# kakaobrain/hqtransformer

Hardware: AMD Instinct MI355X
Metric: images/sec (256x256 class-cond sampling) (higher is better)
Workload: dtype bf16

## Files before the change

hqtransformer_amd/_lib.py:

```python
from __future__ import annotations

import ctypes as C
import os
import subprocess
from typing import List, Optional

HERE = os.path.dirname(os.path.abspath(__file__))
LIB_PATH = os.path.join(HERE, 'libhqt.so')
CSRC = os.path.join(HERE, 'csrc')
SOURCES = ['engine.hip', 'kernels.hip', 'attention.hip', 'fast_kernels.hip', 'persist.hip', 'tile_gemm.hip', 'exact_gemm.hip', 'mfma_gemm.hip', 'split_conv.hip', 'split_stream_conv.hip']
ABI_VERSION = 9

PRECISION_EXACT, PRECISION_FAST, PRECISION_SPLIT = 0, 1, 2
PRECISIONS = {'exact': PRECISION_EXACT, 'fast': PRECISION_FAST, 'split': PRECISION_SPLIT}
POLICY_LATENCY, POLICY_THROUGHPUT = 0, 1
SWITCH_PERSIST, SWITCH_SINGLE_KEY, SWITCH_PERSIST_FAULT, SWITCH_SPLIT_KSLICES = 0, 1, 2, 3
LAYOUT_FAST, LAYOUT_EXACT, LAYOUT_SPLIT, LAYOUT_ALL = 1, 2, 4, 7
RESAMPLE_PIXELSHUFFLE, RESAMPLE_NEAREST, RESAMPLE_CONV2 = 0, 1, 2


class HqtLibraryError(RuntimeError):
    pass


class HqtError(RuntimeError):
    def __init__(self, code: int, msg: str):
        super().__init__(f'libhqt error {code}: {msg}')
        self.code = code


class hqt_config(C.Structure):
# ... 78 lines not shown
    'hqt_decode_seq': (C.c_int, [_VP, C.c_int, _I64P, _I64P, _F32P, C.c_int, C.c_int, _VP]),
    'hqt_sample_l3': (C.c_int, [_VP, C.c_int, _I64P, C.POINTER(hqt_sample_opts_l3), _F32P, _I64P, _I64P, _I64P, _F32P, _I64P, _I64P, _I64P, _VP]),
    'hqt_sample_prefix_l3': (C.c_int, [_VP, C.c_int, _I64P, C.POINTER(hqt_sample_opts_l3), _F32P, C.c_int, _I64P, _I64P, _I64P, _I64P, _I64P, _I64P, _F32P, _I64P, _I64P, _I64P, _VP]),
    'hqt_decode_l3': (C.c_int, [_VP, C.c_int, _I64P, _I64P, _I64P, _F32P, C.c_int, C.c_int, _VP]),
    'hqt_decode_seq_l3': (C.c_int, [_VP, C.c_int, _I64P, _I64P, _I64P, _F32P, C.c_int, C.c_int, _VP]),
    'hqt_encode': (C.c_int, [_VP, C.c_int, _F32P, C.c_int, C.POINTER(hqt_encode_out), _VP]),
    'hqt_has_encoder': (C.c_int, [_VP]),
    'hqt_range_check': (C.c_int, [_VP, _VP]),
    'hqt_param_count': (C.c_int64, [_VP, C.c_int]),
    'hqt_workspace_bytes': (C.c_int64, [_VP]),
    'hqt_timing_enable': (C.c_int, [_VP, C.c_int]),
    'hqt_timing_reset': (C.c_int, [_VP]),
    'hqt_timing_get': (C.c_int, [_VP, C.c_int, C.c_char_p, C.c_int, C.POINTER(C.c_int64), C.POINTER(C.c_double)]),
    'hqt_timing_slots': (C.c_int, [_VP]),
    'hqt_destroy': (C.c_int, [_VP]),
}

_lib: Optional[C.CDLL] = None


def build(force: bool = False, verbose: bool = False) -> str:
    import hashlib
    from concurrent.futures import ThreadPoolExecutor
    hdrs = sorted([os.path.join(CSRC, f) for f in os.listdir(CSRC) if f.endswith('.h')] + [os.path.join(os.path.dirname(HERE), 'include', 'hqt.h')])
    hipcc = os.environ.get('HIPCC', '/opt/rocm/bin/hipcc')
    flags = ['-O3', '--offload-arch=gfx950', '-std=c++17', '-fPIC', '-Wno-unused-value', '-Wno-unused-result']
    objdir = os.path.join(CSRC, 'build')
    os.makedirs(objdir, exist_ok=True)
    ver = subprocess.run([hipcc, '--version'], stdout=subprocess.PIPE, stderr=subprocess.STDOUT, text=True).stdout
    common = hashlib.sha256()
# ... 134 lines not shown
```

hqtransformer_amd/csrc/common.h:

```cpp
#pragma once
#include <hip/hip_runtime.h>
#include <stdint.h>
#include <string>

typedef uint16_t bf16_t;

__device__ __host__ inline float bf16_to_f32(bf16_t v) {
    union { uint32_t u; float f; } c;
    c.u = ((uint32_t)v) << 16;
    return c.f;
}
__device__ __forceinline__ void bf16x8_to_f32(const uint4& raw, float (&f)[8]) {
    const unsigned w[4] = {raw.x, raw.y, raw.z, raw.w};
#pragma unroll
    for (int i = 0; i < 4; ++i) { f[2 * i] = bf16_to_f32((bf16_t)(w[i] & 0xffffu)); f[2 * i + 1] = bf16_to_f32((bf16_t)(w[i] >> 16)); }
}
__device__ __host__ inline bf16_t f32_to_bf16(float f) {
#if defined(__HIP_DEVICE_COMPILE__)
    return __builtin_bit_cast(bf16_t, (__bf16)f);
#endif
    union { uint32_t u; float f; } c;
    c.f = f;
    if ((c.u & 0x7fffffffu) > 0x7f800000u) return (bf16_t)((c.u >> 16) | 0x40);
    return (bf16_t)((c.u + 0x7fffu + ((c.u >> 16) & 1u)) >> 16);
// ... 104 lines not shown
    const float* ln_colsum;
    float ln_eps;
    bf16_t* resid_pk;
    float* resid_parts;
    unsigned* tile_ctr;
    const float* am_rownorm;
    const float* am_colnorm;
    unsigned long long* am_best;
    ChainSync chain;
    float* gn_part_out;
    int gn_out_groups;
    int tune;
    const void* Bw_lo;
    const void* Bw_frag16;
    const void* Bw_up16;
    double* gn_part_out_d;
    int a_f32;
    int b_f32;
    int* range_flag;
    int out_split;
    int k_quarters;
    int b_tile16;
    int k_slices;
    float* k_slabs;
    int tile_panel;
};

struct StepState {
    int step;
    int t_base;
// ... 19 lines not shown
```

hqtransformer_amd/csrc/engine.hip:

```cpp
#include "../../include/hqt.h"
#include "kernels.h"
#include "fast_kernels.h"
#include "split_kernels.h"
#include "persist.h"

#include <algorithm>
#include <cmath>
#include <cstdarg>
#include <cstdio>
#include <cstring>
#include <map>
#include <memory>
#include <mutex>
#include <string>
#include <vector>

static thread_local std::string g_err;
static int fail(int code, const char* fmt, ...) {
    char buf[1024];
    va_list ap;
    va_start(ap, fmt);
    vsnprintf(buf, sizeof(buf), fmt, ap);
    va_end(ap);
    g_err = buf;
// ... 28 lines not shown
struct Tensor {
    float* d = nullptr;
    std::vector<int64_t> shape;
    size_t n = 0;
};

struct Lin {
    const float* w32 = nullptr;
    const float* b32 = nullptr;
    bf16_t* w16 = nullptr;
    half_t* w16h = nullptr;
    half_t* w16l = nullptr;
    float* w32t = nullptr;
    half_t* wfrag16 = nullptr;
    half_t* wup16 = nullptr;
    bf16_t* wpk = nullptr;
    bf16_t* wpk_ln = nullptr;
    float* colsum = nullptr;
    float* bias_ln = nullptr;
    int N = 0, K = 0;
};

struct BlockW {
    bool body = false;
    const float *ln1_g, *ln1_b, *ln2_g, *ln2_b;
    Lin qkv, proj, fc1, fc2;
};

struct DecLayer {
    int kind;
// ... 88 lines not shown
    hipGraphExec_t graph_exec = nullptr;
    std::vector<uint64_t> graph_key;
    hqt_handle* parent = nullptr;
    int n_clones = 0;
    int policy = 0;
    PersistProg pbody, pfull;
    float* lnf_shift = nullptr;
    int ncu = 0;
    unsigned* persist_counters = nullptr;
    unsigned* persist_err = nullptr;
    float* persist_slabs = nullptr;
    bool persist_used = false;
    bool persist_enabled = true;
    bool persist_tripped = false;
    bool single_key = true;
    bool split_kslices = true;
    bool capture_persist = false;
    bool graph_has_persist = false;
    int layouts = 0;
    bool timing = false;
    std::vector<TimingSlot> slots;
    hipEvent_t chain_ev = nullptr;
    bool chain_valid = false;
    std::vector<hipEvent_t> all_events;
};

static int dev_alloc(hqt_handle* h, void** p, size_t bytes, bool workspace) {
    HIPCHK(hipMalloc(p, bytes ? bytes : 16));
    const bool poison = getenv("HQT_POISON_WORKSPACE") != nullptr;
    if (poison && workspace && bytes) HIPCHK(hipMemset(*p, 0xFF, bytes));
// ... 141 lines not shown
extern "C" const char* hqt_last_error(void) { return g_err.c_str(); }

static int alloc_workspace(hqt_handle* hp);

extern "C" int hqt_create(const hqt_config* cfg, int device, hqt_handle** out) {
    if (!cfg || !out) return fail(HQT_ERR_INVALID, "null argument");
    if (cfg->abi_version != HQT_ABI_VERSION) return fail(HQT_ERR_INVALID, "abi_version %d != %d", cfg->abi_version, HQT_ABI_VERSION);
    if (cfg->max_batch < 1) return fail(HQT_ERR_INVALID, "max_batch must be >= 1");
    DeviceGuard dg(device);
    if (!dg.ok) return fail(HQT_ERR_HIP, "hipSetDevice(%d) failed", device);
    std::unique_ptr<hqt_handle> h(new hqt_handle());
    h->tile_gemm = getenv("HQT_NO_TILE_GEMM") == nullptr;
    { const char* e = getenv("HQT_PERSIST"); h->persist_enabled = !(e && atoi(e) == 0); }
    h->single_key = getenv("HQT_NO_SINGLE_KEY") == nullptr;
    h->split_kslices = getenv("HQT_SPLIT_KSLICES_OFF") == nullptr;
    h->cfg = *cfg;
    h->layouts = (cfg->ar_layouts & HQT_LAYOUT_ALL) ? (cfg->ar_layouts & HQT_LAYOUT_ALL) : HQT_LAYOUT_ALL;
    h->device = device;
    const hqt_config& c = h->cfg;
    if (c.has_stage2) {
        if (c.embed_dim % c.n_heads || c.embed_dim % 16) return fail(HQT_ERR_INVALID, "embed_dim must be a multiple of n_heads and 16");
        const int hs = c.embed_dim / c.n_heads;
        if (hs % 8 || hs > 256 || (hs & (hs - 1))) return fail(HQT_ERR_INVALID, "head_dim %d unsupported (power of two in [8, 256])", hs);
        if (c.vocab_top != c.vocab_bot) return fail(HQT_ERR_INVALID, "vocab_top != vocab_bot");
        const bool bidir = c.depth_decoding == HQT_DEPTH_BIDIRECTIONAL;
        if (c.depth_decoding < 0 || c.depth_decoding > HQT_DEPTH_BIDIRECTIONAL || (c.depth_decoding && !bidir && c.code_levels != 3) || (bidir && c.code_levels == 3))
            return fail(HQT_ERR_INVALID, "depth_decoding %d: 0 'parallel-add', 1 'parallel', 2 'parallel-reduce', 3 'top2mid2bot' (three code levels only), "
                        "4 'bidirectional' (two code levels only)", c.depth_decoding);
        if (bidir && c.cond_type == HQT_COND_TEXT)
            return fail(HQT_ERR_INVALID, "depth_decoding 4 'bidirectional' with text conditioning is not built");
// ... 278 lines not shown
    *out = it->second.d;
    return HQT_OK;
}

static int make_lin(hqt_handle* h, Lin& l, const float* w32, const float* b32, int N, int K, bool stream_pack, bool split_planes = false) {
    l.w32 = w32; l.b32 = b32; l.N = N; l.K = K;
    if (!stream_pack || (h->layouts & HQT_LAYOUT_FAST)) {
        CHK(dev_alloc(h, (void**)&l.w16, (size_t)N * K * 2, false));
        HIPCHK(launch_f32_to_bf16(w32, l.w16, (size_t)N * K, 0));
    }
    const bool ar = stream_pack;
    if (split_planes && (!ar || (h->layouts & HQT_LAYOUT_SPLIT))) {
        CHK(dev_alloc(h, (void**)&l.w16h, (size_t)N * K * 2, false));
        CHK(dev_alloc(h, (void**)&l.w16l, (size_t)N * K * 2, false));
        HIPCHK(launch_split_f32(w32, l.w16h, l.w16l, (size_t)N * K, 0));
    }
    if (stream_pack && (h->layouts & HQT_LAYOUT_EXACT) && N % 16 == 0 && K % 32 == 0) {
        CHK(dev_alloc(h, (void**)&l.w32t, (size_t)N * K * 4, false));
        HIPCHK(launch_pack_exact_tiles(w32, l.w32t, N, K, 0));
    }
    if (stream_pack && (h->layouts & HQT_LAYOUT_FAST) && stream_gemm_supported(N, K)) {
        CHK(dev_alloc(h, (void**)&l.wpk, (size_t)N * K * 2, false));
        HIPCHK(launch_pack_stream_weights(w32, l.wpk, N, K, 0));
    }
    return HQT_OK;
}

static int fold_ln(hqt_handle* h, Lin& l, const float* gamma, const float* beta) {
    if (!l.wpk) return HQT_OK;
    CHK(dev_alloc(h, (void**)&l.wpk_ln, (size_t)l.N * l.K * 2, false));
// ... 241 lines not shown
            else if (l.kind == 1) {
                CHK(get_w(h, "stage1." + l.name + ".norm1.weight", {l.cin}, &l.n1_g));
                CHK(get_w(h, "stage1." + l.name + ".norm1.bias", {l.cin}, &l.n1_b));
                CHK(get_w(h, "stage1." + l.name + ".norm2.weight", {l.cout}, &l.n2_g));
                CHK(get_w(h, "stage1." + l.name + ".norm2.bias", {l.cout}, &l.n2_b));
                CHK(load_conv(h, l.name + ".conv1", l.cout, l.cin, 3, l.conv1));
                CHK(load_conv(h, l.name + ".conv2", l.cout, l.cout, 3, l.conv2));
                if (l.cin != l.cout) CHK(load_conv(h, l.name + ".nin_shortcut", l.cout, l.cin, 1, l.nin));
            } else if (l.kind == 2) {
                CHK(get_w(h, "stage1." + l.name + ".norm.weight", {l.cin}, &l.n1_g));
                CHK(get_w(h, "stage1." + l.name + ".norm.bias", {l.cin}, &l.n1_b));
                CHK(load_conv(h, l.name + ".q", l.cin, l.cin, 1, l.q));
                CHK(load_conv(h, l.name + ".k", l.cin, l.cin, 1, l.k));
                CHK(load_conv(h, l.name + ".v", l.cin, l.cin, 1, l.v));
                CHK(load_conv(h, l.name + ".proj_out", l.cin, l.cin, 1, l.proj));
            } else {
                CHK(get_w(h, "stage1.decoder.norm_out.weight", {l.cin}, &l.n1_g));
                CHK(get_w(h, "stage1.decoder.norm_out.bias", {l.cin}, &l.n1_b));
                CHK(load_conv(h, "decoder.conv_out", l.cout, l.cin, 3, l.conv1));
            }
        }
    }
    if (c.has_stage1 && h->w.count("stage1.encoder.conv_in.weight") && (c.s1_resample != HQT_RESAMPLE_CONV2 || h->w.count("stage1.down_t.weight")))
        CHK(load_encoder(h));
    HIPCHK(stream_gemm_configure());
    HIPCHK(tile_gemm_configure());
    HIPCHK(mfma_gemm_configure());
    HIPCHK(split_kernels_configure());
    HIPCHK(hipDeviceSynchronize());
    h->finalized = true;
    return HQT_OK;
// ... 9 lines not shown
static int mode_of(int precision, bool stage1, Mode* md) {
    if (precision == HQT_PRECISION_FAST) md->fast = true;
    else if (precision == HQT_PRECISION_SPLIT && stage1) md->split = true;
    else if (precision == HQT_PRECISION_SPLIT) md->split_ar = true;
    else if (precision != HQT_PRECISION_EXACT) return fail(HQT_ERR_INVALID, "unknown precision %d", precision);
    return HQT_OK;
}

static void lin_args(const hqt_handle* h, GemmArgs& g, const Lin& l, bool split_planes) {
    g.N = l.N; g.K = l.K; g.ldb = l.K;
    g.bias = l.b32;
    g.zero_page = h->zero_page;
    g.tune = h->policy;
    if (g.alpha == 0.0f) g.alpha = 1.0f;
    if (g.lda == 0) g.lda = l.K;
    if (split_planes) { g.Bw = l.w16h; g.Bw_lo = l.w16l; g.Bw_frag16 = l.wfrag16; g.Bw_up16 = l.wup16; }
}

struct SlotName {
    char s[64];
    SlotName(const char* tag, int rows) {
        static const bool by_rows = getenv("HQT_TIMING_BY_ROWS") != nullptr;
        snprintf(s, sizeof s, by_rows ? "%s@%d" : "%s", tag, rows);
    }
};

static int ar_linear(hqt_handle* h, const Mode& md, GemmArgs g, const Lin& l, int a_dt, int c_dt, hipStream_t st,
                     const char* tag, bool defer_residual = false, int* resid_nparts = nullptr) {
    lin_args(h, g, l, false);
    g.k_quarters = 1;
    const SlotName slot(tag, g.M);
// ... 28 lines not shown
            count_variant(h, "variant:stream_gemm:%s", tag);
            if (S > 1) h->pend = {h->splitk, S, 32 * g.a_packed_mb, l.b32};
            return HQT_OK;
        }
        g.Bw = l.w16;
        if (mfma_gemm_ok(g, a_dt, DT_BF16, c_dt)) HIPCHK(launch_mfma_gemm(g, a_dt, DT_BF16, c_dt, st));
        else HIPCHK(launch_gemm_generic(g, a_dt, DT_BF16, c_dt, st));
        return HQT_OK;
    }
    if (md.split_ar && l.w16h && l.w16l && !g.a_packed_mb && g.M > 256) {
        GemmArgs sg = g;
        lin_args(h, sg, l, true);
        sg.a_f32 = 1; sg.range_flag = h->range_flag;
        if (split_gemm_ok(sg)) {
            const int S = h->split_kslices ? split_gemm_slices(sg) : 1;
            if (S > 1 && (size_t)S * sg.M * sg.N <= h->splitk_elems) { sg.k_slices = S; sg.k_slabs = h->splitk; }
            HIPCHK(launch_split_gemm(sg, st));
            if (sg.k_slices > 1) count_variant(h, "variant:split_gemm_kslices%d:%s", sg.k_slices, tag);
            else count_variant(h, "variant:split_gemm:%s", tag);
            return HQT_OK;
        }
    }
    g.Bw = l.w32;
    if (exact_mfma_ok(g)) {
        if (l.w32t && g.N % 16 == 0) { g.Bw = l.w32t; g.b_tile16 = 1; }
        HIPCHK(launch_exact_mfma_gemm(g, st));
        count_variant(h, "variant:exact_mfma:%s", tag);
        return HQT_OK;
    }
    HIPCHK(launch_gemm_generic(g, DT_F32, DT_F32, DT_F32, st));
// ... 853 lines not shown
            Timed t(h, "embed_prefix", c.st);
            HIPCHK(launch_embed_prefix(embed_args(h, c, own), P + 1, P + 1, 0, 0, c.st));
        }
        CHK(run_position(h, c, P + 1, 0, false));
        HIPCHK(launch_advance_step(h->state, P + 1, c.st));
        first = P + 1;
    }
    const int remaining = c.n_steps - first;
    if (remaining <= 0) return HQT_OK;
    if (c.use_graph && !h->timing) {
        static const int gmax = getenv("HQT_GRAPH_POSITIONS") ? std::max(1, atoi(getenv("HQT_GRAPH_POSITIONS"))) : 16;
        int G = 1;
        for (int d = std::min(gmax, remaining); d >= 1; --d) if (remaining % d == 0) { G = d; break; }
        std::vector<uint64_t> key = {(uint64_t)G, (uint64_t)B, (uint64_t)(c.cond != nullptr), (uint64_t)c.noise, (uint64_t)c.logits_out, (uint64_t)c.logprob_out,
                                     (uint64_t)c.precision, (uint64_t)c.n_steps, (uint64_t)c.levels, (uint64_t)h->policy,
                                     (uint64_t)((h->persist_enabled && !h->persist_tripped ? 1 : 0) + (h->single_key ? 0 : 4) + (h->split_kslices ? 0 : 8))};
        for (const int64_t* f : c.feed) key.push_back((uint64_t)f);
        for (const SamplerSet& l : c.lv) {
            uint32_t f[2];
            memcpy(f, &l.top_p, 4); memcpy(f + 1, &l.temperature, 4);
            key.push_back((uint64_t)l.top_k); key.push_back(f[0]); key.push_back(f[1]);
        }
        key.push_back((uint64_t)((c.row_set ? 1 : 0) + (c.row_top_p ? 2 : 0)));
        key.push_back((uint64_t)c.n_guide);
        if (!h->graph_exec || key != h->graph_key) {
            if (h->graph_exec) {
                HIPCHK(hipStreamSynchronize(c.st));
                hipGraphExecDestroy(h->graph_exec);
                h->graph_exec = nullptr;
            }
            hipStream_t cs;
// ... 115 lines not shown
            g->a_f32 = 1; g->range_flag = c.h->range_flag; *a = S1_SPLIT_IN_KERNEL;
            return HQT_OK;
        }
    }
    if (!split_shape_ok(c.h, *g, l)) return HQT_OK;
    *a = S1_PLANES;
    return s1_split_pack(c, g, nullptr, nullptr, nullptr, 0);
}

static int s1_conv(S1Ctx& c, GemmArgs g, S1Operand a, const Lin& l, int c_dt, const char* tag) {
    hqt_handle* h = c.h;
    lin_args(h, g, l, a != S1_TENSOR);
    Timed t(h, SlotName(tag, g.M).s, c.st);
    if (c.gn_ready.tensor == g.C) c.gn_ready.tensor = nullptr;
    if (a != S1_TENSOR) {
        if (g.conv_taps != 9) { HIPCHK(launch_split_gemm(g, c.st)); return HQT_OK; }
        if (g.store == STORE_ROWS && h->gn_tiles && conv_halo_stats_ok(g.N, 32)) {
            g.gn_part_out_d = reinterpret_cast<double*>(h->gn_tiles); g.gn_out_groups = 32;
            c.gn_ready = {g.C, split_conv3_tiles_per_image(g), true};
        }
        HIPCHK(launch_split_conv3(g, c.st));
        return HQT_OK;
    }
    if (c.md.fast) {
        g.Bw = l.w16;
        if (!mfma_gemm_ok(g, c.adt, DT_BF16, c_dt)) { HIPCHK(launch_gemm_generic(g, c.adt, DT_BF16, c_dt, c.st)); return HQT_OK; }
        if (g.conv_taps == 9 && g.store == STORE_ROWS && h->gn_tiles && conv_halo_ok(g, c_dt) && conv_halo_stats_ok(g.N, 32) &&
            !getenv("HQT_NO_FUSED_GN")) {
            g.gn_part_out = h->gn_tiles; g.gn_out_groups = 32;
            c.gn_ready = {g.C, conv_halo_tiles_per_image(g), false};
        }
// ... 315 lines not shown
        }
        { Timed t(h, "vq_finish", st); HIPCHK(launch_vq_finish(a, st)); }
        if (out->diff) HIPCHK(launch_vq_diff(a.err_rows, M, 0.25f / ((float)M * (float)dim), out->diff + l, st));
    }
    if (out->recon) HIPCHK(launch_nhwc_to_nchw_f32(h->vq_recon, out->recon, B, r * r, E, st));
    return HQT_OK;
}

extern "C" int hqt_set_policy(hqt_handle* h, int policy) {
    if (!h) return fail(HQT_ERR_INVALID, "null handle");
    if (policy != HQT_POLICY_LATENCY && policy != HQT_POLICY_THROUGHPUT) return fail(HQT_ERR_INVALID, "unknown policy %d", policy);
    h->policy = policy;
    return HQT_OK;
}

extern "C" int hqt_set_switch(hqt_handle* h, int which, int on) {
    if (!h) return fail(HQT_ERR_INVALID, "null handle");
    if (which == HQT_SWITCH_PERSIST) { h->persist_enabled = on != 0; if (on) h->persist_tripped = false; }
    else if (which == HQT_SWITCH_SINGLE_KEY) h->single_key = on != 0;
    else if (which == HQT_SWITCH_SPLIT_KSLICES) h->split_kslices = on != 0;
    else if (which == HQT_SWITCH_PERSIST_FAULT) {
        if (!h->persist_err) return fail(HQT_ERR_STATE, "no persistent chain on this handle (a lane, or a handle without stage 2)");
        ON_DEVICE(h);
        const unsigned v = (unsigned)on;
        HIPCHK(hipDeviceSynchronize());
        HIPCHK(hipMemcpy(h->persist_err + 1, &v, sizeof v, hipMemcpyHostToDevice));
    }
    else return fail(HQT_ERR_INVALID, "unknown switch %d", which);
    return HQT_OK;
}

extern "C" int hqt_range_check(hqt_handle* h, void* stream) {
    if (!h) return fail(HQT_ERR_INVALID, "null");
    ON_DEVICE(h);
    int flag = 0;
// ... 39 lines not shown
```

hqtransformer_amd/csrc/split_conv.hip:

```cpp
#include "split_kernels.h"
#include "split_ring.h"
#include "gemm_generic.h"
#include <algorithm>
#include <cstdlib>
#include <type_traits>

namespace {
__device__ __forceinline__ unsigned pack_h2(half_t a, half_t b) {
    return (unsigned)__builtin_bit_cast(unsigned short, a) | ((unsigned)__builtin_bit_cast(unsigned short, b) << 16);
}

__device__ __forceinline__ void xcd_tile(int& tile_m, int& tile_n) {
    const int nx = gridDim.x, total = gridDim.x * gridDim.y;
    int id = blockIdx.x + nx * blockIdx.y;
    if ((total & 7) == 0) id = (id & 7) * (total >> 3) + (id >> 3);
    tile_m = id / nx;
    tile_n = id - tile_m * nx;
}
}

__global__ void split_f32_kernel(const float* __restrict__ src, half_t* __restrict__ hi, half_t* __restrict__ lo, size_t n) {
    for (size_t i = blockIdx.x * (size_t)blockDim.x + threadIdx.x; i < n; i += (size_t)gridDim.x * blockDim.x) split2(src[i], hi[i], lo[i]);
}
hipError_t launch_split_f32(const float* src, half_t* hi, half_t* lo, size_t n, hipStream_t st) {
// ... 689 lines not shown
    const int S = g.k_slices > 1 ? g.k_slices : 1;
    const dim3 grid((g.N + 127) / 128, (g.M + 127) / 128, S > 1 ? S : (g.batch > 0 ? g.batch : 1));
    if (g.a_f32 && g.b_f32) split_gemm_kernel<true, true><<<grid, 256, 2 * 4 * 128 * 64, st>>>(g, a_lo_off);
    else if (g.a_f32) split_gemm_kernel<true, false><<<grid, 256, 2 * 4 * 128 * 64, st>>>(g, a_lo_off);
    else split_gemm_kernel<false, false><<<grid, 256, 2 * 4 * 128 * 64, st>>>(g, a_lo_off);
    if (S > 1) {
        const long long n = (long long)g.M * (g.N / 4);
        split_rows_combine_kernel<<<(unsigned)((n + 255) / 256), 256, 0, st>>>(reinterpret_cast<float*>(g.C), g.ldc, reinterpret_cast<const float*>(g.resid), g.k_slabs, g.bias, g.M, g.N, S, g.act);
    }
    return hipGetLastError();
}

hipError_t split_kernels_configure() {
    hipError_t e = split_stream_configure();
    if (e != hipSuccess) return e;
    e = hipFuncSetAttribute(reinterpret_cast<const void*>(conv3x3_split_kernel<false, 128, 1>), hipFuncAttributeMaxDynamicSharedMemorySize, split_conv3_lds(128));
    if (e != hipSuccess) return e;
    e = hipFuncSetAttribute(reinterpret_cast<const void*>(conv3x3_split_kernel<true, 32, 1>), hipFuncAttributeMaxDynamicSharedMemorySize, split_conv3_lds(32));
    if (e != hipSuccess) return e;
    e = hipFuncSetAttribute(reinterpret_cast<const void*>(split_gemm_kernel<true, true>), hipFuncAttributeMaxDynamicSharedMemorySize, 2 * 4 * 128 * 64);
    if (e != hipSuccess) return e;
    e = hipFuncSetAttribute(reinterpret_cast<const void*>(split_gemm_kernel<true, false>), hipFuncAttributeMaxDynamicSharedMemorySize, 2 * 4 * 128 * 64);
    if (e != hipSuccess) return e;
    return hipFuncSetAttribute(reinterpret_cast<const void*>(split_gemm_kernel<false, false>), hipFuncAttributeMaxDynamicSharedMemorySize, 2 * 4 * 128 * 64);
}
```

hqtransformer_amd/csrc/split_kernels.h:

```cpp
#pragma once
#include "common.h"
#include "kernels.h"

typedef _Float16 half_t;

hipError_t launch_split_f32(const float* src, half_t* hi, half_t* lo, size_t n, hipStream_t st);

hipError_t launch_split_pack(const float* x, half_t* y, const float* stats, const float* gamma, const float* beta, int B, int HW,
                             int C, int groups, int swish, int* range_flag, hipStream_t st);

bool split_conv3_ok(const GemmArgs& g);
bool split_gemm_ok(const GemmArgs& g);
hipError_t launch_split_conv3(const GemmArgs& g, hipStream_t st);
hipError_t launch_split_gemm(const GemmArgs& g, hipStream_t st);
int split_gemm_slices(const GemmArgs& g);
int split_conv3_tiles_per_image(const GemmArgs& g);
hipError_t split_kernels_configure();

size_t split_frag_elems(int N, int Cin);
hipError_t launch_pack_split_frag16(const float* w_tapmajor, half_t* out, int N, int Cin, hipStream_t st);
size_t split_up_elems(int N, int Cin);
hipError_t launch_pack_split_up16(const float* w_tapmajor, half_t* out, int N, int Cin, hipStream_t st);
bool split_stream_ok(const GemmArgs& g);
bool split_conv3_emits_planes(const GemmArgs& g);
int split_stream_tiles_per_image(const GemmArgs& g);
hipError_t launch_split_conv3_stream(const GemmArgs& g, hipStream_t st);
hipError_t split_stream_configure();
bool conv_out_direct_ok(const GemmArgs& g);
hipError_t launch_conv_out_direct(const GemmArgs& g, hipStream_t st);
```

hqtransformer_amd/engine.py:

```python
from __future__ import annotations

import ctypes as C
import weakref
from typing import Dict, List, Optional, Sequence, Tuple

import numpy as np
import torch

from . import _lib
from ._lib import PRECISION_EXACT, PRECISION_FAST, hqt_config, hqt_encode_out, hqt_guide_pair, hqt_row_sampler, hqt_sample_opts, hqt_sample_opts_l3
from .spec import DEPTH_DECODINGS, STAGE1_RESAMPLES, Stage1Spec, Stage2Spec


def _ptr(t: Optional[torch.Tensor]) -> Optional[int]:
    return None if t is None else t.data_ptr()


def make_config(s2: Optional[Stage2Spec], s1: Optional[Stage1Spec], max_batch: int, max_steps: int, ar_layouts: int = 0) -> hqt_config:
    c = hqt_config()
    c.abi_version = _lib.ABI_VERSION
    c.max_batch = int(max_batch)
    c.max_steps = int(max_steps)
    c.ar_layouts = int(ar_layouts)
    if s2 is not None:
# ... 177 lines not shown
        e._parent = self
        self._clones = getattr(self, '_clones', [])
        self._clones.append(e)
        return e

    def set_policy(self, policy: int) -> None:
        _lib.check(self.lib.hqt_set_policy(self.h, int(policy)))
        self.policy = int(policy)

    def set_persist(self, on: bool) -> None:
        _lib.check(self.lib.hqt_set_switch(self.h, _lib.SWITCH_PERSIST, int(bool(on))))

    def set_persist_fault(self, cu_plus_one: int) -> None:
        with torch.cuda.device(self.device):
            _lib.check(self.lib.hqt_set_switch(self.h, _lib.SWITCH_PERSIST_FAULT, int(cu_plus_one)))

    def set_split_kslices(self, on: bool) -> None:
        _lib.check(self.lib.hqt_set_switch(self.h, _lib.SWITCH_SPLIT_KSLICES, int(bool(on))))

    def set_single_key(self, on: bool) -> None:
        _lib.check(self.lib.hqt_set_switch(self.h, _lib.SWITCH_SINGLE_KEY, int(bool(on))))

    def _note_split(self, precision: int, stream: int, ar_rows: int = 0) -> None:
        if int(precision) == _lib.PRECISION_SPLIT or (int(precision) == _lib.PRECISION_FAST and 0 < ar_rows <= 64):
            self._split_streams = getattr(self, '_split_streams', set()) | {int(stream or 0)}

    def range_check(self) -> None:
        streams, self._split_streams = getattr(self, '_split_streams', set()), set()
        err = None
        with torch.cuda.device(self.device):
# ... 313 lines not shown
```

include/hqt.h:

```cpp
#ifndef HQT_H
#define HQT_H

#include <stdint.h>

#ifdef __cplusplus
extern "C" {
#endif

#define HQT_ABI_VERSION 9

typedef enum {
    HQT_OK = 0,
    HQT_ERR_INVALID = -1,
    HQT_ERR_HIP = -2,
    HQT_ERR_STATE = -3,
    HQT_ERR_UNKNOWN_WEIGHT = -4,
    HQT_ERR_SHAPE = -5,
    HQT_ERR_MISSING_WEIGHT = -6,
    HQT_ERR_RANGE = -7
} hqt_status;

enum { HQT_COND_NONE = 0, HQT_COND_CLASS = 1, HQT_COND_TEXT = 2 };
enum { HQT_EMB_TRANSFORMER1 = 0, HQT_EMB_REDUCE = 1 };
enum { HQT_PRECISION_EXACT = 0, HQT_PRECISION_FAST = 1, HQT_PRECISION_SPLIT = 2 };
// ... 48 lines not shown
    const uint64_t* row_seeds;
    const int64_t* row_offsets;
} hqt_sample_opts;

int hqt_create(const hqt_config* cfg, int device, hqt_handle** out);

int hqt_set_weight(hqt_handle* h, const char* name, const void* data, int dtype, const int64_t* shape, int ndim);

int hqt_finalize_weights(hqt_handle* h);

int hqt_clone(hqt_handle* src, hqt_handle** out);

enum { HQT_POLICY_LATENCY = 0, HQT_POLICY_THROUGHPUT = 1 };
int hqt_set_policy(hqt_handle* h, int policy);

enum { HQT_SWITCH_PERSIST = 0, HQT_SWITCH_SINGLE_KEY = 1, HQT_SWITCH_PERSIST_FAULT = 2, HQT_SWITCH_SPLIT_KSLICES = 3 };
int hqt_set_switch(hqt_handle* h, int which, int on);

typedef struct { float temperature[3]; int32_t top_k[3]; float top_p[3]; } hqt_row_sampler;
int hqt_set_row_samplers(hqt_handle* h, int n, const hqt_row_sampler* rows);

int hqt_set_logprob_out(hqt_handle* h, float* logprobs);

typedef struct { int32_t pos_row, neg_row; float scale[3]; } hqt_guide_pair;
int hqt_set_guidance(hqt_handle* h, int n_pairs, const hqt_guide_pair* pairs);

int hqt_sample(hqt_handle* h, int B, const int64_t* cond, const hqt_sample_opts* opts, const float* noise,
               const int64_t* force_top, const int64_t* force_bot, float* logits_out,
               int64_t* out_top, int64_t* out_bot, void* stream);

typedef struct {
    int32_t precision, n_steps;
// ... 63 lines not shown
```

Before: 1696.

## Add row-streaming split-precision GEMM with prepacked weights for large-M 1x1 layers

Adds a split-precision GEMM kernel that reads weights prepacked into an MFMA-fragment order (hi/lo planes interleaved). For small K the whole weight panel stays resident in LDS, and the kernel loops persistently over row blocks with a register ring of A prefetches. Otherwise it streams weight chunks. The engine sends f32-input, unsliced GEMMs with M >= 2048 (decoder 1x1 convs and linear layers) to this kernel by default. The cost is extra device memory for the packed weights and a new dispatch heuristic.

```diff
diff --git a/hqtransformer_amd/_lib.py b/hqtransformer_amd/_lib.py
--- a/hqtransformer_amd/_lib.py
+++ b/hqtransformer_amd/_lib.py
@@ -8,13 +8,13 @@
 HERE = os.path.dirname(os.path.abspath(__file__))
 LIB_PATH = os.path.join(HERE, 'libhqt.so')
 CSRC = os.path.join(HERE, 'csrc')
-SOURCES = ['engine.hip', 'kernels.hip', 'attention.hip', 'fast_kernels.hip', 'persist.hip', 'tile_gemm.hip', 'exact_gemm.hip', 'mfma_gemm.hip', 'split_conv.hip', 'split_stream_conv.hip']
+SOURCES = ['engine.hip', 'kernels.hip', 'attention.hip', 'fast_kernels.hip', 'persist.hip', 'tile_gemm.hip', 'exact_gemm.hip', 'mfma_gemm.hip', 'split_conv.hip', 'split_stream_conv.hip', 'split_rows_gemm.hip']
 ABI_VERSION = 9
 
 PRECISION_EXACT, PRECISION_FAST, PRECISION_SPLIT = 0, 1, 2
 PRECISIONS = {'exact': PRECISION_EXACT, 'fast': PRECISION_FAST, 'split': PRECISION_SPLIT}
 POLICY_LATENCY, POLICY_THROUGHPUT = 0, 1
-SWITCH_PERSIST, SWITCH_SINGLE_KEY, SWITCH_PERSIST_FAULT, SWITCH_SPLIT_KSLICES = 0, 1, 2, 3
+SWITCH_PERSIST, SWITCH_SINGLE_KEY, SWITCH_PERSIST_FAULT, SWITCH_SPLIT_KSLICES, SWITCH_SPLIT_ROWS_GEMM = 0, 1, 2, 3, 4
 LAYOUT_FAST, LAYOUT_EXACT, LAYOUT_SPLIT, LAYOUT_ALL = 1, 2, 4, 7
 RESAMPLE_PIXELSHUFFLE, RESAMPLE_NEAREST, RESAMPLE_CONV2 = 0, 1, 2
 
@@ -123,6 +123,9 @@
     'hqt_timing_get': (C.c_int, [_VP, C.c_int, C.c_char_p, C.c_int, C.POINTER(C.c_int64), C.POINTER(C.c_double)]),
     'hqt_timing_slots': (C.c_int, [_VP]),
     'hqt_destroy': (C.c_int, [_VP]),
+    'hqt_split_rows_probe_ok': (C.c_int, [C.c_int] * 7),
+    'hqt_split_rows_pack_index': (C.c_int64, [C.c_int, C.c_int, C.c_int64, C.POINTER(C.c_int)]),
+    'hqt_split_gemm_probe': (C.c_int, [C.c_int] * 5 + [_VP, _VP, _VP, _VP, _VP, C.c_int, C.POINTER(C.c_int)]),
 }
 
 _lib: Optional[C.CDLL] = None
diff --git a/hqtransformer_amd/csrc/common.h b/hqtransformer_amd/csrc/common.h
--- a/hqtransformer_amd/csrc/common.h
+++ b/hqtransformer_amd/csrc/common.h
@@ -142,6 +142,7 @@
     const void* Bw_lo;
     const void* Bw_frag16;
     const void* Bw_up16;
+    const void* Bw_rows;
     double* gn_part_out_d;
     int a_f32;
     int b_f32;
diff --git a/hqtransformer_amd/csrc/engine.hip b/hqtransformer_amd/csrc/engine.hip
--- a/hqtransformer_amd/csrc/engine.hip
+++ b/hqtransformer_amd/csrc/engine.hip
@@ -66,6 +66,7 @@
     float* w32t = nullptr;
     half_t* wfrag16 = nullptr;
     half_t* wup16 = nullptr;
+    half_t* wrows = nullptr;
     bf16_t* wpk = nullptr;
     bf16_t* wpk_ln = nullptr;
     float* colsum = nullptr;
@@ -184,6 +185,7 @@
     bool persist_enabled = true;
     bool persist_tripped = false;
     bool single_key = true;
+    bool split_rows = true;
     bool split_kslices = true;
     bool capture_persist = false;
     bool graph_has_persist = false;
@@ -355,6 +357,7 @@
     { const char* e = getenv("HQT_PERSIST"); h->persist_enabled = !(e && atoi(e) == 0); }
     h->single_key = getenv("HQT_NO_SINGLE_KEY") == nullptr;
     h->split_kslices = getenv("HQT_SPLIT_KSLICES_OFF") == nullptr;
+    { const char* e = getenv("HQT_SPLIT_ROWS_GEMM"); h->split_rows = !(e && e[0] == '0' && !e[1]); }
     h->cfg = *cfg;
     h->layouts = (cfg->ar_layouts & HQT_LAYOUT_ALL) ? (cfg->ar_layouts & HQT_LAYOUT_ALL) : HQT_LAYOUT_ALL;
     h->device = device;
@@ -663,6 +666,10 @@
         CHK(dev_alloc(h, (void**)&l.w16h, (size_t)N * K * 2, false));
         CHK(dev_alloc(h, (void**)&l.w16l, (size_t)N * K * 2, false));
         HIPCHK(launch_split_f32(w32, l.w16h, l.w16l, (size_t)N * K, 0));
+        if (N % 128 == 0 && K % 64 == 0) {
+            CHK(dev_alloc(h, (void**)&l.wrows, split_rows_elems(N, K) * sizeof(half_t), false));
+            HIPCHK(launch_pack_split_rows(l.w16h, l.w16l, l.wrows, N, K, 0));
+        }
     }
     if (stream_pack && (h->layouts & HQT_LAYOUT_EXACT) && N % 16 == 0 && K % 32 == 0) {
         CHK(dev_alloc(h, (void**)&l.w32t, (size_t)N * K * 4, false));
@@ -934,7 +941,7 @@
                 CHK(load_conv(h, l.name + ".k", l.cin, l.cin, 1, l.k));
                 CHK(load_conv(h, l.name + ".v", l.cin, l.cin, 1, l.v));
                 CHK(load_conv(h, l.name + ".proj_out", l.cin, l.cin, 1, l.proj));
-            } else {
+                } else {
                 CHK(get_w(h, "stage1.decoder.norm_out.weight", {l.cin}, &l.n1_g));
                 CHK(get_w(h, "stage1.decoder.norm_out.bias", {l.cin}, &l.n1_b));
                 CHK(load_conv(h, "decoder.conv_out", l.cout, l.cin, 3, l.conv1));
@@ -974,7 +981,7 @@
     g.tune = h->policy;
     if (g.alpha == 0.0f) g.alpha = 1.0f;
     if (g.lda == 0) g.lda = l.K;
-    if (split_planes) { g.Bw = l.w16h; g.Bw_lo = l.w16l; g.Bw_frag16 = l.wfrag16; g.Bw_up16 = l.wup16; }
+    if (split_planes) { g.Bw = l.w16h; g.Bw_lo = l.w16l; g.Bw_frag16 = l.wfrag16; g.Bw_up16 = l.wup16; g.Bw_rows = h->split_rows ? l.wrows : nullptr; }
 }
 
 struct SlotName {
@@ -1033,6 +1040,11 @@
         sg.a_f32 = 1; sg.range_flag = h->range_flag;
         if (split_gemm_ok(sg)) {
             const int S = h->split_kslices ? split_gemm_slices(sg) : 1;
+            if (S <= 1 && split_rows_gemm_faster(sg)) {
+                HIPCHK(launch_split_rows_gemm(sg, st));
+                count_variant(h, "variant:split_gemm_rows:%s", tag);
+                return HQT_OK;
+            }
             if (S > 1 && (size_t)S * sg.M * sg.N <= h->splitk_elems) { sg.k_slices = S; sg.k_slabs = h->splitk; }
             HIPCHK(launch_split_gemm(sg, st));
             if (sg.k_slices > 1) count_variant(h, "variant:split_gemm_kslices%d:%s", sg.k_slices, tag);
@@ -1916,7 +1928,7 @@
         for (int d = std::min(gmax, remaining); d >= 1; --d) if (remaining % d == 0) { G = d; break; }
         std::vector<uint64_t> key = {(uint64_t)G, (uint64_t)B, (uint64_t)(c.cond != nullptr), (uint64_t)c.noise, (uint64_t)c.logits_out, (uint64_t)c.logprob_out,
                                      (uint64_t)c.precision, (uint64_t)c.n_steps, (uint64_t)c.levels, (uint64_t)h->policy,
-                                     (uint64_t)((h->persist_enabled && !h->persist_tripped ? 1 : 0) + (h->single_key ? 0 : 4) + (h->split_kslices ? 0 : 8))};
+                                     (uint64_t)((h->persist_enabled && !h->persist_tripped ? 1 : 0) + (h->single_key ? 0 : 4) + (h->split_kslices ? 0 : 8) + (h->split_rows ? 0 : 16))};
         for (const int64_t* f : c.feed) key.push_back((uint64_t)f);
         for (const SamplerSet& l : c.lv) {
             uint32_t f[2];
@@ -2062,7 +2074,13 @@
     Timed t(h, SlotName(tag, g.M).s, c.st);
     if (c.gn_ready.tensor == g.C) c.gn_ready.tensor = nullptr;
     if (a != S1_TENSOR) {
-        if (g.conv_taps != 9) { HIPCHK(launch_split_gemm(g, c.st)); return HQT_OK; }
+        if (g.conv_taps != 9) {
+            if (split_rows_gemm_faster(g)) {
+                HIPCHK(launch_split_rows_gemm(g, c.st));
+                count_variant(h, "variant:split_gemm_rows:%s", tag);
+            } else HIPCHK(launch_split_gemm(g, c.st));
+            return HQT_OK;
+        }
         if (g.store == STORE_ROWS && h->gn_tiles && conv_halo_stats_ok(g.N, 32)) {
             g.gn_part_out_d = reinterpret_cast<double*>(h->gn_tiles); g.gn_out_groups = 32;
             c.gn_ready = {g.C, split_conv3_tiles_per_image(g), true};
@@ -2408,11 +2426,58 @@
     return HQT_OK;
 }
 
+extern "C" int hqt_split_rows_probe_ok(int M, int N, int K, int a_f32, int b_f32, int batch, int k_slices) {
+    static const char dummy[16] = {0};
+    GemmArgs g{};
+    g.A = dummy; g.Bw = dummy; g.Bw_lo = dummy; g.Bw_rows = dummy; g.zero_page = dummy; g.C = const_cast<char*>(dummy);
+    g.M = M; g.N = N; g.K = K; g.lda = a_f32 ? K : 2 * K; g.ldb = K; g.ldc = N; g.a_f32 = a_f32; g.b_f32 = b_f32; g.batch = batch; g.k_slices = k_slices;
+    g.alpha = 1.0f; g.store = STORE_ROWS;
+    return (split_rows_gemm_ok(g) ? 1 : 0) | (split_rows_gemm_faster(g) ? 2 : 0);
+}
+extern "C" long long hqt_split_rows_pack_index(int N, int K, long long i, int* plane) { return split_rows_pack_index(N, K, i, plane); }
+extern "C" int hqt_split_gemm_probe(int rows_kernel, int M, int N, int K, int a_f32, const void* A, const float* W, const float* bias, const float* resid, float* C,
+                                    int rows_per_image, int* range_flag_out) {
+    if (M <= 0 || N <= 0 || K <= 0 || !A || !W || !C) return fail(HQT_ERR_INVALID, "hqt_split_gemm_probe: bad arguments");
+    half_t *wh = nullptr, *wl = nullptr, *wr = nullptr;
+    char* zero = nullptr;
+    int rc = HQT_OK;
+    auto body = [&]() -> int {
+        HIPCHK(split_kernels_configure());
+        HIPCHK(hipMalloc((void**)&wh, (size_t)N * K * 2));
+        HIPCHK(hipMalloc((void**)&wl, (size_t)N * K * 2));
+        HIPCHK(hipMalloc((void**)&zero, 512));
+        HIPCHK(hipMemset(zero, 0, 512));
+        HIPCHK(launch_split_f32(W, wh, wl, (size_t)N * K, 0));
+        GemmArgs g{};
+        g.A = A; g.a_f32 = a_f32; g.lda = a_f32 ? K : 2 * K; g.Bw = wh; g.Bw_lo = wl; g.ldb = K; g.C = C; g.ldc = N; g.M = M; g.N = N; g.K = K; g.batch = 1;
+        g.bias = bias; g.resid = resid; g.alpha = 1.0f; g.zero_page = zero; g.range_flag = reinterpret_cast<int*>(zero + 256);
+        g.store = rows_per_image > 0 ? STORE_NCHW : STORE_ROWS; g.rows_per_image = rows_per_image;
+        if (rows_kernel) {
+            if (N % 128 != 0 || K % 16 != 0) return fail(HQT_ERR_INVALID, "hqt_split_gemm_probe: shape not packable");
+            HIPCHK(hipMalloc((void**)&wr, split_rows_elems(N, K) * sizeof(half_t)));
+            HIPCHK(launch_pack_split_rows(wh, wl, wr, N, K, 0));
+            g.Bw_rows = wr;
+            if (!split_rows_gemm_ok(g)) return fail(HQT_ERR_INVALID, "hqt_split_gemm_probe: split_rows_gemm_kernel does not take this shape");
+            HIPCHK(launch_split_rows_gemm(g, 0));
+        } else {
+            if (!split_gemm_ok(g)) return fail(HQT_ERR_INVALID, "hqt_split_gemm_probe: split_gemm_kernel does not take this shape");
+            HIPCHK(launch_split_gemm(g, 0));
+        }
+        HIPCHK(hipDeviceSynchronize());
+        if (range_flag_out) HIPCHK(hipMemcpy(range_flag_out, zero + 256, sizeof(int), hipMemcpyDeviceToHost));
+        return HQT_OK;
+    };
+    rc = body();
+    hipFree(wh); hipFree(wl); hipFree(wr); hipFree(zero);
+    return rc;
+}
+
 extern "C" int hqt_set_switch(hqt_handle* h, int which, int on) {
     if (!h) return fail(HQT_ERR_INVALID, "null handle");
     if (which == HQT_SWITCH_PERSIST) { h->persist_enabled = on != 0; if (on) h->persist_tripped = false; }
     else if (which == HQT_SWITCH_SINGLE_KEY) h->single_key = on != 0;
     else if (which == HQT_SWITCH_SPLIT_KSLICES) h->split_kslices = on != 0;
+    else if (which == HQT_SWITCH_SPLIT_ROWS_GEMM) h->split_rows = on != 0;
     else if (which == HQT_SWITCH_PERSIST_FAULT) {
         if (!h->persist_err) return fail(HQT_ERR_STATE, "no persistent chain on this handle (a lane, or a handle without stage 2)");
         ON_DEVICE(h);
diff --git a/hqtransformer_amd/csrc/split_conv.hip b/hqtransformer_amd/csrc/split_conv.hip
--- a/hqtransformer_amd/csrc/split_conv.hip
+++ b/hqtransformer_amd/csrc/split_conv.hip
@@ -727,6 +727,8 @@
 hipError_t split_kernels_configure() {
     hipError_t e = split_stream_configure();
     if (e != hipSuccess) return e;
+    e = split_rows_configure();
+    if (e != hipSuccess) return e;
     e = hipFuncSetAttribute(reinterpret_cast<const void*>(conv3x3_split_kernel<false, 128, 1>), hipFuncAttributeMaxDynamicSharedMemorySize, split_conv3_lds(128));
     if (e != hipSuccess) return e;
     e = hipFuncSetAttribute(reinterpret_cast<const void*>(conv3x3_split_kernel<true, 32, 1>), hipFuncAttributeMaxDynamicSharedMemorySize, split_conv3_lds(32));
diff --git a/hqtransformer_amd/csrc/split_kernels.h b/hqtransformer_amd/csrc/split_kernels.h
--- a/hqtransformer_amd/csrc/split_kernels.h
+++ b/hqtransformer_amd/csrc/split_kernels.h
@@ -15,6 +15,15 @@
 hipError_t launch_split_gemm(const GemmArgs& g, hipStream_t st);
 int split_gemm_slices(const GemmArgs& g);
 int split_conv3_tiles_per_image(const GemmArgs& g);
+constexpr int SPLIT_ROWS_MIN_M = 2048;
+size_t split_rows_elems(int N, int K);
+long long split_rows_pack_index(int N, int K, long long i, int* plane);
+hipError_t launch_pack_split_rows(const half_t* hi, const half_t* lo, half_t* out, int N, int K, hipStream_t st);
+bool split_rows_gemm_ok(const GemmArgs& g);
+bool split_rows_gemm_faster(const GemmArgs& g);
+bool split_rows_gemm_resident(const GemmArgs& g);
+hipError_t launch_split_rows_gemm(const GemmArgs& g, hipStream_t st);
+hipError_t split_rows_configure();
 hipError_t split_kernels_configure();
 
 size_t split_frag_elems(int N, int Cin);
diff --git a/hqtransformer_amd/csrc/split_rows_gemm.hip b/hqtransformer_amd/csrc/split_rows_gemm.hip
--- /dev/null
+++ b/hqtransformer_amd/csrc/split_rows_gemm.hip
@@ -0,0 +1,298 @@
+#include "split_kernels.h"
+#include "split_device.h"
+#include "split_ring.h"
+#include "gemm_generic.h"
+#include <algorithm>
+
+namespace {
+constexpr int SRG_BN = 128;
+constexpr int SRG_STEP = 8192;
+constexpr int SRG_CHUNK = 4 * SRG_STEP;
+constexpr int SRG_PITCH = 32 + 4;
+constexpr int SRG_PATCH = 32 * SRG_PITCH * 4;
+constexpr int SRG_TAIL = SRG_BN * 4 + 4 * SRG_PATCH;
+}
+
+__host__ __device__ inline size_t split_rows_src(size_t i, int K, int& plane) {
+    const int KS = K / 16;
+    const int e = (int)(i & 7), lane = (int)((i >> 3) & 63);
+    size_t ch = i >> 9;
+    plane = (int)(ch & 1); ch >>= 1;
+    const int j = (int)(ch & 3); ch >>= 2;
+    const int s = (int)(ch % KS);
+    const int tn = (int)(ch / KS);
+    return (size_t)(tn * SRG_BN + j * 32 + (lane & 31)) * K + s * 16 + 8 * (lane >> 5) + e;
+}
+__global__ void pack_split_rows_kernel(const half_t* __restrict__ hi, const half_t* __restrict__ lo, half_t* __restrict__ out, int K, size_t total) {
+    for (size_t i = blockIdx.x * (size_t)blockDim.x + threadIdx.x; i < total; i += (size_t)gridDim.x * blockDim.x) {
+        int plane;
+        const size_t src = split_rows_src(i, K, plane);
+        out[i] = plane ? lo[src] : hi[src];
+    }
+}
+long long split_rows_pack_index(int N, int K, long long i, int* plane) {
+    if (N <= 0 || K <= 0 || N % SRG_BN != 0 || K % 16 != 0 || i < 0 || (size_t)i >= split_rows_elems(N, K)) return -1;
+    return (long long)split_rows_src((size_t)i, K, *plane);
+}
+size_t split_rows_elems(int N, int K) { return (size_t)N * K * 2; }
+hipError_t launch_pack_split_rows(const half_t* hi, const half_t* lo, half_t* out, int N, int K, hipStream_t st) {
+    const size_t total = split_rows_elems(N, K);
+    pack_split_rows_kernel<<<(int)std::min<size_t>((total + 255) / 256, 8192), 256, 0, st>>>(hi, lo, out, K, total);
+    return hipGetLastError();
+}
+
+#ifndef SRG_RING_RESIDENT
+#define SRG_RING_RESIDENT 8
+#endif
+#ifndef SRG_RING_STREAMED
+#define SRG_RING_STREAMED 4
+#endif
+template <bool AF32, bool RESIDENT, int R = RESIDENT ? SRG_RING_RESIDENT : SRG_RING_STREAMED>
+__global__ __launch_bounds__(256, RESIDENT ? 1 : 2) void split_rows_gemm_kernel(GemmArgs g, int a_lo_off, int row_blocks) {
+    extern __shared__ __attribute__((aligned(16))) char lds_raw[];
+    const int tid = threadIdx.x, lane = tid & 63, wave = __builtin_amdgcn_readfirstlane(tid >> 6);
+    const int fr = lane & 31, fh = lane >> 5;
+    const int KS = g.K / 16, NCH = KS / 4;
+    static_assert(R % 4 == 0, "whole filter chunks");
+    const int n0 = blockIdx.x * SRG_BN;
+    const char* wsrc = reinterpret_cast<const char*>(g.Bw_rows) + (size_t)blockIdx.x * KS * SRG_STEP;
+    char* const tail = RESIDENT ? lds_raw + (size_t)KS * SRG_STEP : lds_raw;
+    float* const lbias = reinterpret_cast<float*>(tail);
+    float* const patch = reinterpret_cast<float*>(tail + SRG_BN * 4 + wave * SRG_PATCH);
+    const char* zero = reinterpret_cast<const char*>(g.zero_page);
+    const int rb_stride = RESIDENT ? (int)gridDim.y * 4 : 1;
+    int rb = (int)blockIdx.y * 4 + wave;
+
+    auto a_row = [&](int b) -> const char* {
+        const long long m = (long long)b * 32 + fr;
+        if (b >= row_blocks || m >= g.M) return nullptr;
+        return reinterpret_cast<const char*>(g.A) + (m * g.lda + fh * 8) * (AF32 ? 4 : 2);
+    };
+    auto fetch = [&](u32x4 (&sl)[2], const char* row, int s) {
+        if (AF32) {
+            const char* p = row ? row + s * 64 : zero;
+            sl[0] = *reinterpret_cast<const u32x4*>(p);
+            sl[1] = *reinterpret_cast<const u32x4*>(p + 16);
+        } else {
+            sl[0] = *reinterpret_cast<const u32x4*>(row ? row + s * 32 : zero);
+            sl[1] = *reinterpret_cast<const u32x4*>(row ? row + s * 32 + a_lo_off * 2 : zero);
+        }
+    };
+#ifdef HQT_SPLIT_GEMM_STAMPS
+    long long st_pro = clock64(), st_loop = 0, st_epi = 0;
+#endif
+    const char* pa = a_row(rb);
+    u32x4 ring[R][2];
+#pragma unroll
+    for (int u = 0; u < R; ++u) fetch(ring[u], pa, u);
+    if (RESIDENT) {
+        const int total = KS * SRG_STEP;
+        for (int off = tid * 16; off < total; off += 8 * 4096) {
+            u32x4 w[8];
+#pragma unroll
+            for (int p = 0; p < 8; ++p) w[p] = *reinterpret_cast<const u32x4*>(wsrc + off + p * 4096);
+#pragma unroll
+            for (int p = 0; p < 8; ++p) *reinterpret_cast<u32x4*>(lds_raw + off + p * 4096) = w[p];
+        }
+        if (tid < SRG_BN) lbias[tid] = g.bias ? g.bias[n0 + tid] : 0.0f;
+    } else {
+#pragma unroll
+        for (int p = 0; p < 8; ++p) *reinterpret_cast<u32x4*>(lds_raw + tid * 16 + p * 4096) = *reinterpret_cast<const u32x4*>(wsrc + tid * 16 + p * 4096);
+    }
+    __syncthreads();
+#ifdef HQT_SPLIT_GEMM_STAMPS
+    st_pro = clock64() - st_pro;
+#endif
+    bool bad = false;
+    float* const C0 = reinterpret_cast<float*>(g.C);
+    const float* const Rb = g.resid ? reinterpret_cast<const float*>(g.resid) : nullptr;
+
+    for (int it = 0; RESIDENT ? rb < row_blocks : it < 1; ++it, rb += rb_stride) {
+#ifdef HQT_SPLIT_GEMM_STAMPS
+        const long long t0 = clock64();
+#endif
+        const char* pan = RESIDENT ? a_row(rb + rb_stride) : nullptr;
+        f32x16 accm[4], accx[4];
+#pragma unroll
+        for (int j = 0; j < 4; ++j)
+#pragma unroll
+            for (int r = 0; r < 16; ++r) { accm[j][r] = 0.0f; accx[j][r] = 0.0f; }
+        for (int c0 = 0; c0 < NCH; c0 += R / 4) {
+            u32x4 wst[8];
+#pragma unroll
+            for (int u = 0; u < R; ++u) {
+                const int c = c0 + u / 4;
+                if (!RESIDENT && u % 4 == 0) {
+                    const char* src = wsrc + (size_t)min(c + 1, NCH - 1) * SRG_CHUNK + tid * 16;
+#pragma unroll
+                    for (int p = 0; p < 8; ++p) wst[p] = *reinterpret_cast<const u32x4*>(src + p * 4096);
+                }
+                const char* wl = lds_raw + (RESIDENT ? (size_t)c * SRG_CHUNK : (size_t)(c & 1) * SRG_CHUNK) + lane * 16;
+                half8 ah, al;
+                if (AF32) {
+                    float xs[8];
+#pragma unroll
+                    for (int e = 0; e < 8; ++e) {
+                        const unsigned bits = ring[u][e >> 2][e & 3];
+                        xs[e] = __builtin_bit_cast(float, bits);
+                    }
+                    unsigned hi[4], lo[4];
+                    split8_checked(xs, hi, lo, bad);
+                    ah = __builtin_bit_cast(half8, u32x4{hi[0], hi[1], hi[2], hi[3]});
+                    al = __builtin_bit_cast(half8, u32x4{lo[0], lo[1], lo[2], lo[3]});
+                } else {
+                    ah = __builtin_bit_cast(half8, ring[u][0]);
+                    al = __builtin_bit_cast(half8, ring[u][1]);
+                }
+                const int sn = c0 * 4 + u + R;
+                fetch(ring[u], sn < KS ? pa : pan, sn < KS ? sn : sn - KS);
+                const char* ws = wl + (u % 4) * SRG_STEP;
+#pragma unroll
+                for (int j = 0; j < 4; ++j) {
+                    const half8 wh = *reinterpret_cast<const half8*>(ws + (j * 2) * 1024);
+                    const half8 wlo = *reinterpret_cast<const half8*>(ws + (j * 2 + 1) * 1024);
+                    accm[j] = __builtin_amdgcn_mfma_f32_32x32x16_f16(wh, ah, accm[j], 0, 0, 0);
+                    accx[j] = __builtin_amdgcn_mfma_f32_32x32x16_f16(wh, al, accx[j], 0, 0, 0);
+                    accx[j] = __builtin_amdgcn_mfma_f32_32x32x16_f16(wlo, ah, accx[j], 0, 0, 0);
+                }
+                if (!RESIDENT && u % 4 == 3) {
+                    char* dst = lds_raw + (size_t)((c + 1) & 1) * SRG_CHUNK + tid * 16;
+#pragma unroll
+                    for (int p = 0; p < 8; ++p) *reinterpret_cast<u32x4*>(dst + p * 4096) = wst[p];
+                    __syncthreads();
+                }
+            }
+        }
+#ifdef HQT_SPLIT_GEMM_STAMPS
+        const long long t1 = clock64();
+        st_loop += t1 - t0;
+#endif
+        if (!RESIDENT) {
+            if (tid < SRG_BN) lbias[tid] = g.bias ? g.bias[n0 + tid] : 0.0f;
+            __syncthreads();
+        }
+        const int mrow0 = rb * 32;
+        const int ncol = n0;
+        float* const Cw = C0;
+        const bool nchw = g.store == STORE_NCHW;
+        const int ncols_dst = g.N;
+        if (!nchw) {
+            const int cg = (lane & 7) * 4, r0 = lane >> 3;
+            f32x4 rs[4][4];
+            if (Rb) {
+#pragma unroll
+                for (int j = 0; j < 4; ++j)
+#pragma unroll
+                    for (int p = 0; p < 4; ++p) {
+                        const long long m = min((long long)mrow0 + p * 8 + r0, (long long)g.M - 1);
+                        rs[j][p] = *reinterpret_cast<const f32x4*>(Rb + m * g.ldc + ncol + j * 32 + cg);
+                    }
+            }
+            dispatch_act(g.act, [&](auto act_c) {
+            constexpr int ACT = decltype(act_c)::value;
+#pragma unroll
+            for (int j = 0; j < 4; ++j) {
+#pragma unroll
+                for (int q4 = 0; q4 < 4; ++q4) {
+                    const int cl = 8 * q4 + 4 * fh;
+                    const f32x4 bq = *reinterpret_cast<const f32x4*>(lbias + j * 32 + cl);
+                    f32x4 v;
+#pragma unroll
+                    for (int e = 0; e < 4; ++e) v[e] = apply_act_c<ACT>((accm[j][4 * q4 + e] + accx[j][4 * q4 + e] * SPLIT_INV) * g.alpha + bq[e]);
+                    *reinterpret_cast<f32x4*>(patch + fr * SRG_PITCH + cl) = v;
+                }
+                __builtin_amdgcn_fence(__ATOMIC_ACQ_REL, "wavefront");
+                __builtin_amdgcn_wave_barrier();
+#pragma unroll
+                for (int p = 0; p < 4; ++p) {
+                    const int r = p * 8 + r0;
+                    const long long m = (long long)mrow0 + r;
+                    f32x4 v = *reinterpret_cast<const f32x4*>(patch + r * SRG_PITCH + cg);
+                    if (Rb) v += rs[j][p];
+                    if (m < g.M) *reinterpret_cast<f32x4*>(Cw + m * g.ldc + ncol + j * 32 + cg) = v;
+                }
+                __builtin_amdgcn_fence(__ATOMIC_ACQ_REL, "wavefront");
+                __builtin_amdgcn_wave_barrier();
+            }
+            });
+        } else {
+            const long long m = (long long)mrow0 + fr;
+            if (m < g.M) {
+                const int img = (int)(m / g.rows_per_image), pix = (int)(m - (long long)img * g.rows_per_image);
+#pragma unroll
+                for (int j = 0; j < 4; ++j)
+#pragma unroll
+                    for (int q4 = 0; q4 < 4; ++q4) {
+                        const int nl = j * 32 + 8 * q4 + 4 * fh;
+                        const f32x4 bq = *reinterpret_cast<const f32x4*>(lbias + nl);
+                        float s[4];
+#pragma unroll
+                        for (int e = 0; e < 4; ++e) s[e] = accm[j][4 * q4 + e] + accx[j][4 * q4 + e] * SPLIT_INV;
+#pragma unroll
+                        for (int e = 0; e < 4; ++e) {
+                            float x = s[e] * g.alpha + bq[e];
+                            if (g.clamp01) x = fminf(fmaxf(0.5f * x + 0.5f, 0.0f), 1.0f);
+                            Cw[((long long)img * ncols_dst + ncol + nl + e) * g.rows_per_image + pix] = x;
+                        }
+                    }
+            }
+        }
+        pa = pan;
+#ifdef HQT_SPLIT_GEMM_STAMPS
+        st_epi += clock64() - t1;
+#endif
+    }
+    if (AF32 && bad && g.range_flag) atomicOr(g.range_flag, 1);
+#ifdef HQT_SPLIT_GEMM_STAMPS
+    if (g.am_best && tid == 0) {
+        long long* d = reinterpret_cast<long long*>(g.am_best) + (size_t)(blockIdx.x + gridDim.x * blockIdx.y) * 4;
+        d[0] = st_pro; d[1] = st_loop; d[2] = st_epi; d[3] = wall_clock64();
+    }
+#endif
+}
+
+bool split_rows_gemm_ok(const GemmArgs& g) {
+    if (!g.Bw_rows || !g.zero_page || g.b_f32 || g.batch > 1 || g.k_slices > 1) return false;
+    if (g.gn_stats || g.a_packed_mb || g.a_rows_per_group || g.conv_taps > 1 || g.conv_stride2 || g.upsample) return false;
+    if (g.K % (16 * SRG_RING_STREAMED) != 0 || g.N % SRG_BN != 0 || g.M <= 0) return false;
+    const int lda = g.conv_taps ? (g.a_f32 ? g.Cin : 2 * g.Cin) : g.lda;
+    if (lda % (g.a_f32 ? 4 : 8) != 0) return false;
+    if (g.store == STORE_NCHW) return !g.resid && g.act == ACT_NONE && g.rows_per_image > 0;
+    return g.store == STORE_ROWS && g.rows_per_group == 0 && g.ldc % 4 == 0;
+}
+bool split_rows_gemm_faster(const GemmArgs& g) { return g.a_f32 && g.M >= SPLIT_ROWS_MIN_M && split_rows_gemm_ok(g); }
+bool split_rows_gemm_resident(const GemmArgs& g) { return g.K <= 256 && g.K % (16 * SRG_RING_RESIDENT) == 0; }
+static int split_rows_lds(const GemmArgs& g) { return split_rows_gemm_resident(g) ? (g.K / 16) * SRG_STEP + SRG_TAIL : 2 * SRG_CHUNK; }
+
+hipError_t launch_split_rows_gemm(const GemmArgs& g0, hipStream_t st) {
+    GemmArgs g = g0;
+    if (g.conv_taps == 1) { g.lda = g.a_f32 ? g.Cin : 2 * g.Cin; g.conv_taps = 0; }
+    const int a_lo_off = g.lda / 2;
+    const int row_blocks = (g.M + 31) / 32, tiles = (row_blocks + 3) / 4, nt = g.N / SRG_BN;
+    if (split_rows_gemm_resident(g)) {
+        static int cus = 0;
+        if (!cus) {
+            int dev = 0;
+            if (hipGetDevice(&dev) != hipSuccess || hipDeviceGetAttribute(&cus, hipDeviceAttributeMultiprocessorCount, dev) != hipSuccess || cus <= 0) cus = 256;
+        }
+        const dim3 grid(nt, std::min(tiles, std::max(1, cus / nt)), 1);
+        if (g.a_f32) split_rows_gemm_kernel<true, true><<<grid, 256, split_rows_lds(g), st>>>(g, a_lo_off, row_blocks);
+        else split_rows_gemm_kernel<false, true><<<grid, 256, split_rows_lds(g), st>>>(g, a_lo_off, row_blocks);
+    } else {
+        const dim3 grid(nt, tiles, 1);
+        if (g.a_f32) split_rows_gemm_kernel<true, false><<<grid, 256, split_rows_lds(g), st>>>(g, a_lo_off, row_blocks);
+        else split_rows_gemm_kernel<false, false><<<grid, 256, split_rows_lds(g), st>>>(g, a_lo_off, row_blocks);
+    }
+    return hipGetLastError();
+}
+
+hipError_t split_rows_configure() {
+    const int res = 16 * SRG_STEP + SRG_TAIL;
+    hipError_t e = hipFuncSetAttribute(reinterpret_cast<const void*>(split_rows_gemm_kernel<true, true>), hipFuncAttributeMaxDynamicSharedMemorySize, res);
+    if (e != hipSuccess) return e;
+    e = hipFuncSetAttribute(reinterpret_cast<const void*>(split_rows_gemm_kernel<false, true>), hipFuncAttributeMaxDynamicSharedMemorySize, res);
+    if (e != hipSuccess) return e;
+    e = hipFuncSetAttribute(reinterpret_cast<const void*>(split_rows_gemm_kernel<true, false>), hipFuncAttributeMaxDynamicSharedMemorySize, 2 * SRG_CHUNK);
+    if (e != hipSuccess) return e;
+    return hipFuncSetAttribute(reinterpret_cast<const void*>(split_rows_gemm_kernel<false, false>), hipFuncAttributeMaxDynamicSharedMemorySize, 2 * SRG_CHUNK);
+}
diff --git a/hqtransformer_amd/engine.py b/hqtransformer_amd/engine.py
--- a/hqtransformer_amd/engine.py
+++ b/hqtransformer_amd/engine.py
@@ -215,6 +215,9 @@
     def set_persist_fault(self, cu_plus_one: int) -> None:
         with torch.cuda.device(self.device):
             _lib.check(self.lib.hqt_set_switch(self.h, _lib.SWITCH_PERSIST_FAULT, int(cu_plus_one)))
+
+    def set_split_rows_gemm(self, on: bool) -> None:
+        _lib.check(self.lib.hqt_set_switch(self.h, _lib.SWITCH_SPLIT_ROWS_GEMM, int(bool(on))))
 
     def set_split_kslices(self, on: bool) -> None:
         _lib.check(self.lib.hqt_set_switch(self.h, _lib.SWITCH_SPLIT_KSLICES, int(bool(on))))
diff --git a/include/hqt.h b/include/hqt.h
--- a/include/hqt.h
+++ b/include/hqt.h
@@ -86,8 +86,13 @@
 enum { HQT_POLICY_LATENCY = 0, HQT_POLICY_THROUGHPUT = 1 };
 int hqt_set_policy(hqt_handle* h, int policy);
 
-enum { HQT_SWITCH_PERSIST = 0, HQT_SWITCH_SINGLE_KEY = 1, HQT_SWITCH_PERSIST_FAULT = 2, HQT_SWITCH_SPLIT_KSLICES = 3 };
+enum { HQT_SWITCH_PERSIST = 0, HQT_SWITCH_SINGLE_KEY = 1, HQT_SWITCH_PERSIST_FAULT = 2, HQT_SWITCH_SPLIT_KSLICES = 3, HQT_SWITCH_SPLIT_ROWS_GEMM = 4 };
 int hqt_set_switch(hqt_handle* h, int which, int on);
+
+int hqt_split_rows_probe_ok(int M, int N, int K, int a_f32, int b_f32, int batch, int k_slices);
+long long hqt_split_rows_pack_index(int N, int K, long long i, int* plane);
+int hqt_split_gemm_probe(int rows_kernel, int M, int N, int K, int a_f32, const void* A, const float* W, const float* bias, const float* resid, float* C,
+                         int rows_per_image, int* range_flag_out);
 
 typedef struct { float temperature[3]; int32_t top_k[3]; float top_p[3]; } hqt_row_sampler;
 int hqt_set_row_samplers(hqt_handle* h, int n, const hqt_row_sampler* rows);
```

After: 1704 (median of 6 runs). About the same (+0.5%).
